# liuzuxin/OSRL

Hardware: AMD Instinct MI355X
Metric: grad-steps/sec (higher is better)
Workload: dtype f32

## Files before the change

### osrl_amd/csrc/mlp.hip

```cpp
#include "dwt.h"
#include "adam.h"
#include "gather.h"
#include "step.h"
#include "trace.h"

namespace {


template <int RW, int CNT, int STAGES, int RD>
__device__ __forceinline__ void mm_prefetch(f32x4 (&b)[RD][RW], int nk, const float* __restrict__ P, int Np, int col0,
                                            int kc0 = 0) {
  static_assert(CNT <= RW && STAGES <= RD, "ring too small");
  const int lane = threadIdx.x & 63;
  const unsigned lane_off = (unsigned)(((lane >> 4) * Np + col0 + (lane & 15)) * 16);
  const int rot = k_rot(nk);
#pragma unroll
  for (int s = 0; s < STAGES - 1; ++s) {
    const int kc = k_at(s < nk ? s : nk - 1, rot, nk, kc0);
    const float* __restrict__ Pk = P + (size_t)kc * 16 * Np;
#pragma unroll
    for (int c = 0; c < CNT; ++c) b[s][c] = load_bp_s(Pk, lane_off + c * 256);
  }
}

// ... 137 lines not shown
__device__ __forceinline__ NarrowPart narrow_part(int nk, int col_off, int nblk, int wave) {
  const int parts = NW / nblk;
  const int blk = wave / parts, part = wave - blk * parts;
  const int k_lo = (nk * part) / parts, k_hi = (nk * (part + 1)) / parts;
  return NarrowPart{col_off + blk * 16, k_lo, k_hi - k_lo};
}
template <int NCB, int NW = 4, int RD = kRing>
__device__ __forceinline__ void narrow_prefetch(f32x4 (&ring)[RD][NCB], int nk, const float* __restrict__ P, int Np,
                                                int col_off, int nblk, int wave) {
  const NarrowPart np = narrow_part<NW>(nk, col_off, nblk, wave);
  if (np.k_n > 0) mm_prefetch<NCB, 1, 3>(ring, np.k_n, P, Np, np.col, np.k_lo);
}
template <int NRB, int NCB, int NW = 4, int RD = kRing>
__device__ __forceinline__ void narrow_layer_splitk(float* lds, int lda, int nk, const float* __restrict__ P, int Np,
                                                    int col_off, int nblk, int wave, f32x4 (&ring)[RD][NCB]) {
  const int lane = threadIdx.x & 63;
  const int parts = NW / nblk;
  const NarrowPart np = narrow_part<NW>(nk, col_off, nblk, wave);
  f32x4 t[NRB][1];
#pragma unroll
  for (int rb = 0; rb < NRB; ++rb) t[rb][0] = f32x4{0.f, 0.f, 0.f, 0.f};
  if (np.k_n > 0) mm_run<NRB, 1, NCB, 1, 3>(lds, lda, np.k_n, P, Np, np.col, t, ring, np.k_lo);
  __syncthreads();
  {
    const int ln = fresh_v<NW == 8>(lane), ld = fresh_s<NW == 8>(lda);
#pragma unroll
    for (int rb = 0; rb < NRB; ++rb)
#pragma unroll
      for (int r = 0; r < 4; ++r) lds[(rb * 16 + (ln >> 4) * 4 + r) * ld + wave * 16 + (ln & 15)] = t[rb][0][r];
  }
  __syncthreads();
  constexpr int BM = 16 * NRB;
  const int ncol = nblk * 16;
  float v[(BM * 32 + 64 * NW - 1) / (64 * NW)];
#pragma unroll
  for (int j = 0; j < (BM * 32 + 64 * NW - 1) / (64 * NW); ++j) {
    const int e = j * 64 * NW + (int)threadIdx.x;
    float sacc = 0.f;
    if (e < BM * ncol) {
      const int r = e / ncol, c = e - r * ncol;
      const int b = c >> 4, cc = c & 15;
      for (int q = 0; q < parts; ++q) sacc += lds[r * lda + (b * parts + q) * 16 + cc];
    }
    v[j] = sacc;
  }
  __syncthreads();
#pragma unroll
  for (int j = 0; j < (BM * 32 + 64 * NW - 1) / (64 * NW); ++j) {
    const int e = j * 64 * NW + (int)threadIdx.x;
    if (e < BM * ncol) {
      const int r = e / ncol, c = e - r * ncol;
      lds[r * lda + c] = v[j];
    }
  }
  __syncthreads();
}


template <int NT = 0>
__device__ __forceinline__ void tile_to_global(const float* lds, int lda, int BM, int N, float* __restrict__ dst,
                                               int row0, int rows) {
  const int tid = threadIdx.x;
  if ((N & 3) == 0 && ((reinterpret_cast<uintptr_t>(dst) & 15) == 0)) {
    const int n4 = N >> 2;
    for (int idx = tid; idx < BM * n4; idx += (NT ? NT : (int)blockDim.x)) {
      const int r = idx / n4, c4 = idx - r * n4;
      if (row0 + r < rows)
        *reinterpret_cast<f32x4*>(dst + (size_t)(row0 + r) * N + 4 * c4) =
            *reinterpret_cast<const f32x4*>(lds + r * lda + 4 * c4);
    }
  } else {
    for (int idx = tid; idx < BM * N; idx += (NT ? NT : (int)blockDim.x)) {
      const int r = idx / N, c = idx - r * N;
      if (row0 + r < rows) dst[(size_t)(row0 + r) * N + c] = lds[r * lda + c];
    }
  }
}

template <int NRB, int NCB, int ACT, bool SCALE, bool RAGGED>
__device__ __forceinline__ void fwd_epilogue_core(float* lds, int lda, const f32x4 (&acc)[NRB][NCB], int cb0, int cnt,
                                                  int N, float oscale, int lane) {
#pragma unroll
  for (int c = 0; c < NCB; ++c) {
    if (c < cnt) {
      const int col = (cb0 + c) * 16 + (lane & 15);
      const bool live = col < N;
      float* dst = lds + ((lane >> 4) * 4) * lda + col;
#pragma unroll
      for (int rb = 0; rb < NRB; ++rb) {
#pragma unroll
        for (int r = 0; r < 4; ++r) {
          float v = act_fwd(ACT, acc[rb][c][r]);
          if (SCALE) v *= oscale;
          if (RAGGED) v = live ? v : 0.f;
          dst[(rb * 16 + r) * lda] = v;
        }
      }
    }
  }
}
template <int NRB, int NCB, int ACT>
__device__ __forceinline__ void fwd_epilogue(float* lds, int lda, const f32x4 (&acc)[NRB][NCB], int cb0, int cnt, int N,
                                             float oscale, int lane) {
  if (oscale == 1.0f && (N & 15) == 0)
    fwd_epilogue_core<NRB, NCB, ACT, false, false>(lds, lda, acc, cb0, cnt, N, oscale, lane);
  else
// ... 41 lines not shown
constexpr float kTailLogStdMin = -20.0f, kTailLogStdMax = 2.0f;
template <class TR, int NT = 0>
__device__ __forceinline__ void tail_gauss(const float* lds, int lda, int BM, int row0, int rows, TR t) {
  const int ad = t.L;
  const float max_a = t.max_action;
  const float* __restrict__ e1 = t.eps;
  const float* __restrict__ e2 = t.eps2;
  float* __restrict__ a1 = t.out;
  float* __restrict__ a2 = t.out2;
  float* __restrict__ th2 = t.tanh2;
  for (int idx = threadIdx.x; idx < BM * ad; idx += (NT ? NT : (int)blockDim.x)) {
    const int r = idx / ad, j = idx - r * ad;
    const int gr = row0 + r;
    if (gr < rows) {
      const float mu = lds[r * lda + j];
      const float ls = fminf(fmaxf(lds[r * lda + ad + j], kTailLogStdMin), kTailLogStdMax);
      const float sd = expf(ls);
      const size_t i = (size_t)gr * ad + j;
      if (e1) {
        const float u = mu + sd * e1[i];
        a1[i] = max_a * tanhf(u);
      }
      if (e2) {
        const float u = mu + sd * e2[i];
        const float th = tanhf(u);
        a2[i] = max_a * th;
        if (th2) th2[i] = th;
      }
    }
  }
  const float* __restrict__ eo = t.eps_ood;
  if (eo) {
    float* __restrict__ so = t.out_ood;
    const int ns = t.n_samples;
    for (int idx = threadIdx.x; idx < ns * BM * ad; idx += (NT ? NT : (int)blockDim.x)) {
      const int jr = idx / ad, k = idx - jr * ad;
      const int smp = jr / BM, r = jr - smp * BM;
      const int gr = row0 + r;
      if (gr < rows) {
        const float mu = lds[r * lda + k];
        const float ls = fminf(fmaxf(lds[r * lda + ad + k], kTailLogStdMin), kTailLogStdMax);
        const size_t i = ((size_t)smp * rows + gr) * ad + k;
        so[i] = mu + expf(ls) * eo[i];
      }
    }
  }
}

struct FwdArgs {
  osrl_mlp_t net;
  osrl_rows_t in;
  osrl_mlp_acts_t out;
  int32_t lda;
  osrl_mlp_tail_t tail;
};

#ifndef OSRL_WPS_8
#define OSRL_WPS_8 3
#endif
constexpr int waves_per_simd(int nrb, int ncb) {
  return nrb * ncb >= 14 ? 2 : nrb * ncb == 8 ? OSRL_WPS_8 : nrb * ncb >= 4 ? 3 : 4;
}
#ifndef OSRL_CHAIN_WPS
#define OSRL_CHAIN_WPS 6
#endif
constexpr int chain_wps(int ncb) { return ncb <= 2 ? OSRL_CHAIN_WPS : 2; }
constexpr int waves_per_simd_bwd(int nrb, int ncb) { return nrb * ncb >= 7 ? 2 : 3; }

template <int NRB, int NCB, int NW, class AR>
__device__ __forceinline__ void mlp_fwd_body(AR a, const int e, const int tile) {
  extern __shared__ __attribute__((aligned(16))) float lds[];
  constexpr int BM = 16 * NRB;
  const int tid = threadIdx.x, lane = tid & 63;
  const int wave = __builtin_amdgcn_readfirstlane(tid >> 6);
  const int row0 = tile * BM;
  const int rows = a.in.rows, lda = a.lda;
  const int L = a.net.n_layers;
#if OSRL_CHAIN_PRIO > 0
  if (rows <= OSRL_CHAIN_PRIO) __builtin_amdgcn_s_setprio(3);
#endif

  WG_LOG(0);
  PHASE_STAMP(0);
  f32x4 ring[ring_depth<NW>()][NCB];
  auto begin_layer = [&](int l) {
    const int K = a.net.dims[l], N = a.net.dims[l + 1];
    const int nblk = (N + 15) >> 4, nk = round16(K) >> 4;
    if (nblk <= 2 && nk >= 4 && lda >= 16 * NW) {
      narrow_prefetch<NCB, NW>(ring, nk, a.net.Wf[e][l], round16(N), 0, nblk, wave);
    } else {
      int cb0, cnt;
      wave_blocks<NW>(nblk, wave, &cb0, &cnt);
      layer_prefetch<NRB, NCB>(ring, nk, a.net.Wf[e][l], round16(N), cb0 * 16, cnt);
    }
  };
  begin_layer(0);
  {
    const int K0 = a.net.dims[0], K0p = round16(K0);
    const int d0 = a.in.d0, d1 = a.in.d1;
    const int cl = tid & 15, rl = tid >> 4;
    const float* __restrict__ s0 = a.in.src0;
    const float* __restrict__ s1 = a.in.src1 ? a.in.src1 : a.in.src0;
#pragma unroll 1
    for (int r = rl; r < BM; r += 4 * NW) {
      const int gr = row0 + r;
      const bool rok = gr < rows;
      const int grc = rok ? gr : rows - 1;
      const float* p0 = s0 + (size_t)map_row(grc, a.in.map0, a.in.div0) * d0;
      const float* p1 = s1 + (size_t)map_row(grc, a.in.map1, a.in.div1) * d1 - d0;
      for (int cbase = 0; cbase < K0p; cbase += 16 * 8) {
        float v[8];
#pragma unroll
        for (int j = 0; j < 8; ++j) {
          const int c = cbase + j * 16 + cl;
          const bool in0 = c < d0, ok = rok && c < d0 + d1;
          const float* p = in0 ? p0 + c : p1 + c;
          v[j] = *(ok ? p : s0);
          v[j] = ok ? v[j] : 0.f;
        }
#pragma unroll
        for (int j = 0; j < 8; ++j) {
          const int c = cbase + j * 16 + cl;
          if (c < K0p) lds[r * lda + c] = v[j];
        }
      }
    }
    __syncthreads();
    if (e == 0 && a.out.x) tile_to_global<64 * NW>(lds, lda, BM, K0, a.out.x, row0, rows);
  }
  PHASE_STAMP(1);
  constexpr bool kWarm = OSRL_L2_WARM && NW == 8;
  float warm[OSRL_MAX_LAYERS - 1][kWarmLines];
  if (kWarm) {
    for (int l = 1; l < L; ++l)
      l2_warm<64 * NW>(a.net.Wf[e][l], round16(a.net.dims[l]) * round16(a.net.dims[l + 1]), warm[l - 1]);
  }

  for (int l = 0; l < L; ++l) {
    const int K = a.net.dims[l], N = a.net.dims[l + 1];
    const int nblk = (N + 15) >> 4;
    const float* __restrict__ bias = a.net.b[e][l];
    const int act = a.net.acts[l];
    const float oscale = (l == L - 1) ? a.net.out_scale : 1.0f;
    const int nk = round16(K) >> 4;
    if (nblk <= 2 && nk >= 4 && lda >= 16 * NW) {
      narrow_layer_splitk<NRB, NCB, NW>(lds, lda, nk, a.net.Wf[e][l], round16(N), 0, nblk, wave, ring);
      if (l + 1 < L) begin_layer(l + 1);
      PHASE_STAMP(2 + 4 * l);
      PHASE_STAMP(3 + 4 * l);
      const int ncol = nblk * 16;
      for (int idx = tid; idx < BM * ncol; idx += 64 * NW) {
        const int r = idx / ncol, c = idx - r * ncol;
        const float v = c < N ? act_fwd(act, lds[r * lda + c] + bias[c]) * oscale : 0.f;
        lds[r * lda + c] = v;
      }
    } else {
      int cb0, cnt;
      wave_blocks<NW>(nblk, wave, &cb0, &cnt);
      float bv[NCB];
#pragma unroll
      for (int c = 0; c < NCB; ++c) {
        const int col = (cb0 + c) * 16 + (lane & 15);
        const bool ok = c < cnt && col < N;
        bv[c] = bias[ok ? col : 0];
        bv[c] = ok ? bv[c] : 0.f;
      }
      f32x4 acc[NRB][NCB];
#pragma unroll
      for (int rb = 0; rb < NRB; ++rb)
#pragma unroll
        for (int c = 0; c < NCB; ++c) acc[rb][c] = f32x4{bv[c], bv[c], bv[c], bv[c]};
      if (cnt > 0) layer_run<NRB, NCB>(lds, lda, nk, a.net.Wf[e][l], round16(N), cb0 * 16, cnt, acc, ring);
      if (l + 1 < L) begin_layer(l + 1);
      PHASE_STAMP(2 + 4 * l);
      __syncthreads();
      PHASE_STAMP(3 + 4 * l);
      const int lane_e = fresh_v<NW == 8>(lane), lda_e = fresh_s<NW == 8>(lda);
      if (act == OSRL_ACT_RELU)
        fwd_epilogue<NRB, NCB, OSRL_ACT_RELU>(lds, lda_e, acc, cb0, cnt, N, oscale, lane_e);
      else if (act == OSRL_ACT_TANH)
        fwd_epilogue<NRB, NCB, OSRL_ACT_TANH>(lds, lda_e, acc, cb0, cnt, N, oscale, lane_e);
      else
        fwd_epilogue<NRB, NCB, OSRL_ACT_ID>(lds, lda_e, acc, cb0, cnt, N, oscale, lane_e);
    }
    PHASE_STAMP(4 + 4 * l);
    __syncthreads();
    float* save = a.out.h[e][l];
    if (save) tile_to_global<64 * NW>(lds, lda, BM, N, save, row0, rows);
    PHASE_STAMP(5 + 4 * l);
    if (kWarm && l == 0) {
      for (int w = 1; w < L; ++w) l2_warm_done(warm[w - 1]);
    }
  }
  if (a.tail.kind == OSRL_TAIL_VAE_LATENT && e == 0) tail_vae_latent<decltype((a.tail)), 64 * NW>(lds, lda, BM, row0, rows, a.tail);
  if (a.tail.kind == OSRL_TAIL_GAUSS && e == 0) tail_gauss<decltype((a.tail)), 64 * NW>(lds, lda, BM, row0, rows, a.tail);
  WG_LOG(1);
}

template <int NRB, int NCB, int NW = 4>
__global__ __launch_bounds__(64 * NW, (NW == 8 ? chain_wps(NCB) : waves_per_simd(NRB, NCB))) void mlp_fwd_kernel(const FwdArgs a) {
  mlp_fwd_body<NRB, NCB, NW, const FwdArgs&>(a, blockIdx.y, blockIdx.x);
}
template <int NRB, int NCB, int NW = 4>
__global__ __launch_bounds__(64 * NW, (NW == 8 ? chain_wps(NCB) : waves_per_simd(NRB, NCB))) void mlp_fwd_kernel_p(const void* p) {
  OSRL_TRACE_BEGIN(5, p);
  mlp_fwd_body<NRB, NCB, NW, const OSRL_CAS FwdArgs&>(*(const OSRL_CAS FwdArgs*)p, blockIdx.y, blockIdx.x);
}

template <int NRB, int NCB>
__global__ __launch_bounds__(256, waves_per_simd(NRB, NCB)) void mlp_fwd_loop_kernel(const FwdArgs a) {
  const int n_tiles = (a.in.rows + 16 * NRB - 1) / (16 * NRB);
  for (int tile = blockIdx.x; tile < n_tiles; tile += gridDim.x) {
    mlp_fwd_body<NRB, NCB, 4, const FwdArgs&>(a, blockIdx.y, tile);
    __syncthreads();
  }
}

struct Fwd2Args {
  FwdArgs a0, a1;
  int32_t nets0, tiles0, tiles1, pad_;
};
template <int NRB, int NCB, int NW = 4>
__global__ __launch_bounds__(64 * NW, (NW == 8 ? chain_wps(NCB) : waves_per_simd(NRB, NCB))) void mlp_fwd2_kernel(
    const Fwd2Args f) {
  if ((int)blockIdx.y < f.nets0) {
    if ((int)blockIdx.x >= f.tiles0) return;
    mlp_fwd_body<NRB, NCB, NW, const FwdArgs&>(f.a0, blockIdx.y, blockIdx.x);
  } else {
    if ((int)blockIdx.x >= f.tiles1) return;
    mlp_fwd_body<NRB, NCB, NW, const FwdArgs&>(f.a1, blockIdx.y - f.nets0, blockIdx.x);
  }
}
template <int NRB, int NCB, int NW = 4>
__global__ __launch_bounds__(64 * NW, (NW == 8 ? chain_wps(NCB) : waves_per_simd(NRB, NCB))) void mlp_fwd2_kernel_p(
    const void* p) {
  OSRL_TRACE_BEGIN(6, p);
  const OSRL_CAS Fwd2Args& f = *(const OSRL_CAS Fwd2Args*)p;
  if ((int)blockIdx.y < f.nets0) {
    if ((int)blockIdx.x >= f.tiles0) return;
    mlp_fwd_body<NRB, NCB, NW, const OSRL_CAS FwdArgs&>(f.a0, blockIdx.y, blockIdx.x);
  } else {
    if ((int)blockIdx.x >= f.tiles1) return;
    mlp_fwd_body<NRB, NCB, NW, const OSRL_CAS FwdArgs&>(f.a1, blockIdx.y - f.nets0, blockIdx.x);
  }
// ... 877 lines not shown
    if (RES) rbase = a.resid + (size_t)urow0 * a.ldr + ucol0;
#pragma unroll
    for (int c = 0; c < CB; ++c) pbias[c] = a.bias ? a.bias[ucol0 + c * 16 + (lane & 15)] : 0.f;
#pragma unroll
    for (int r = 0; r < RB; ++r)
#pragma unroll
      for (int c = 0; c < CB; ++c) {
        prev[r][c] = acc[r][c];
        acc[r][c] = f32x4{0.f, 0.f, 0.f, 0.f};
      }
    tile_ptrs(t + 2 < t1 ? t + 2 : t1 - 1, Agn, Bgn);
  }
#pragma unroll
  for (int e = 0; e < 4 * NACC; ++e) {
    float* yp = ybase + el_off(e, (int)a.ldy);
    const int ai = e >> 2, r = ai % RB, c = ai / RB;
    float v = prev[r][c][e & 3] + pbias[c];
    if (RES) v += (rbase + el_off(e, (int)a.ldr))[loff_r];
    yp[loff_y] = v;
  }
  asm volatile("s_waitcnt vmcnt(0)" ::: "memory");
}


__global__ __launch_bounds__(256) void pack_kernel(const float* __restrict__ src_flat, float* __restrict__ pf,
                                                    float* __restrict__ pb, const osrl_pack_entry_t* __restrict__ ents) {
  const osrl_pack_entry_t E = ents[blockIdx.y];
  const float* __restrict__ W = src_flat + E.src_off;
  const int N = E.out, K = E.in;
  const int Np = round16(N), Kp = round16(K);
  if (pf && E.f_off >= 0) {
    float* __restrict__ d = pf + E.f_off;
    const int total = Kp * Np;
    for (int j = blockIdx.x * 256 + threadIdx.x; j < total; j += gridDim.x * 256) {
      const int t = j & 3, n = (j >> 2) % Np, q = (j >> 2) / Np;
      const int k = q * 4 + t;
      d[j] = (n < N && k < K) ? W[(size_t)n * K + k] : 0.f;
    }
  }
  if (pb && E.b_off >= 0) {
    float* __restrict__ d = pb + E.b_off;
    const int Kb = Kp + 16;
    const int total = Np * Kb;
    for (int j = blockIdx.x * 256 + threadIdx.x; j < total; j += gridDim.x * 256) {
      const int t = j & 3, i = (j >> 2) % Kb, q = (j >> 2) / Kb;
      const int o = q * 4 + t;
      d[j] = (o < N && i < K) ? W[(size_t)o * K + i] : 0.f;
    }
  }
}

inline int round16h(int x) { return (x + 15) & ~15; }

struct TileChoice {
  int nrb, ncb, lda, nw;
};

inline TileChoice choose_tile(const osrl_mlp_t* net, int rows, int extra_width) {
  int maxw = extra_width;
  for (int l = 0; l <= net->n_layers; ++l) maxw = net->dims[l] > maxw ? net->dims[l] : maxw;
  const int nblk = (maxw + 15) / 16;
  const int cpw = (nblk + 3) / 4;
  TileChoice t;
  t.ncb = cpw <= 1 ? 1 : cpw <= 2 ? 2 : cpw <= 4 ? 4 : 7;
  t.lda = round16h(maxw) + 8;
  const long wg32 = (long)((rows + 31) / 32) * net->n_nets;
  t.nrb = (t.ncb != 7 && wg32 >= 1024) ? 2 : 1;
  t.nw = 4;
  if (net->tile_rows == 16 || net->tile_rows == 32 || (net->tile_rows == 64 && t.ncb != 7)) {
    t.nrb = net->tile_rows / 16;
    return t;
  }
  const long wg16 = (long)((rows + 15) / 16) * net->n_nets;
  if (t.nrb == 1 && cpw > 2 && wg16 <= 2 * 256 && t.lda >= 128) {
    t.nw = 8;
    t.ncb = (nblk + 7) / 8 <= 2 ? 2 : 4;
  }
  return t;
}

template <typename Args, typename K>
int launch_tiles(K kernel, void (*kernel_p)(const void*), const Args& args, int rows, int nets, int nrb, int lda,
                 hipStream_t stream, int threads = 256, int wg_cap = 0) {
  const int BM = 16 * nrb;
  const size_t lds_bytes = (size_t)BM * lda * sizeof(float);
  int tiles = (rows + BM - 1) / BM;
  if (wg_cap > 0 && tiles * nets > wg_cap) tiles = (wg_cap + nets - 1) / nets;
  return osrl_argmem::launch(kernel, kernel_p, dim3(tiles, nets, 1), dim3(threads), lds_bytes, stream, args);
}
template <typename Args, typename K>
int launch_tiles(K kernel, const Args& args, int rows, int nets, int nrb, int lda, hipStream_t stream,
                 int threads = 256, int wg_cap = 0) {
  return launch_tiles(kernel, (void (*)(const void*))nullptr, args, rows, nets, nrb, lda, stream, threads, wg_cap);
}

#define OSRL_DISPATCH_TILE(KERNEL, ARGS, ROWS, NETS, T, STREAM, CAP)                        \
  do {                                                                                  \
    if (T.nw == 8) {                                                                    \
      if (T.ncb == 2) return launch_tiles(KERNEL<1, 2, 8>, KERNEL##_p<1, 2, 8>, ARGS, ROWS, NETS, 1, T.lda, STREAM, 512, CAP); \
      return launch_tiles(KERNEL<1, 4, 8>, KERNEL##_p<1, 4, 8>, ARGS, ROWS, NETS, 1, T.lda, STREAM, 512, CAP);     \
    }                                                                                   \
    if (T.ncb == 1) {                                                                   \
      if (T.nrb == 4) return launch_tiles(KERNEL<4, 1>, KERNEL##_p<4, 1>, ARGS, ROWS, NETS, 4, T.lda, STREAM, 256, CAP); \
      if (T.nrb == 2) return launch_tiles(KERNEL<2, 1>, KERNEL##_p<2, 1>, ARGS, ROWS, NETS, 2, T.lda, STREAM, 256, CAP); \
      return launch_tiles(KERNEL<1, 1>, KERNEL##_p<1, 1>, ARGS, ROWS, NETS, 1, T.lda, STREAM, 256, CAP);             \
    }                                                                                   \
    if (T.ncb == 2) {                                                                   \
      if (T.nrb == 4) return launch_tiles(KERNEL<4, 2>, KERNEL##_p<4, 2>, ARGS, ROWS, NETS, 4, T.lda, STREAM, 256, CAP); \
      if (T.nrb == 2) return launch_tiles(KERNEL<2, 2>, KERNEL##_p<2, 2>, ARGS, ROWS, NETS, 2, T.lda, STREAM, 256, CAP); \
      return launch_tiles(KERNEL<1, 2>, KERNEL##_p<1, 2>, ARGS, ROWS, NETS, 1, T.lda, STREAM, 256, CAP);             \
    }                                                                                   \
    if (T.ncb == 4) {                                                                   \
      if (T.nrb == 4) return launch_tiles(KERNEL<4, 4>, KERNEL##_p<4, 4>, ARGS, ROWS, NETS, 4, T.lda, STREAM, 256, CAP); \
      if (T.nrb == 2) return launch_tiles(KERNEL<2, 4>, KERNEL##_p<2, 4>, ARGS, ROWS, NETS, 2, T.lda, STREAM, 256, CAP); \
      return launch_tiles(KERNEL<1, 4>, KERNEL##_p<1, 4>, ARGS, ROWS, NETS, 1, T.lda, STREAM, 256, CAP);             \
    }                                                                                   \
    if (T.nrb == 2) return launch_tiles(KERNEL<2, 7>, KERNEL##_p<2, 7>, ARGS, ROWS, NETS, 2, T.lda, STREAM, 256, CAP); \
    return launch_tiles(KERNEL<1, 7>, KERNEL##_p<1, 7>, ARGS, ROWS, NETS, 1, T.lda, STREAM, 256, CAP);               \
  } while (0)

bool valid_net(const osrl_mlp_t* n) {
  if (!n || n->n_layers < 1 || n->n_layers > OSRL_MAX_LAYERS || n->n_nets < 1 || n->n_nets > OSRL_MAX_NETS)
    return false;
  for (int l = 0; l <= n->n_layers; ++l)
    if (n->dims[l] < 1 || n->dims[l] > OSRL_MAX_WIDTH) return false;
  return true;
}

constexpr int kTileMaxWidth = 448;
bool wide_net(const osrl_mlp_t* n) {
  for (int l = 0; l <= n->n_layers; ++l)
    if (n->dims[l] > kTileMaxWidth) return true;
  return false;
}
enum { WIDE_FWD = 0, WIDE_BWD = 1, WIDE_PLAIN = 2 };
struct WideArgs {
  const float* A[OSRL_MAX_NETS];
  const float* P[OSRL_MAX_NETS];
  const float* bias[OSRL_MAX_NETS];
  const float* h[OSRL_MAX_NETS];
  float* Y[OSRL_MAX_NETS];
  osrl_rows_t in;
  float* x;
  int32_t M, K, N, Np, col0, lda, act, mode;
  float oscale;
};
constexpr int kWideMaxK = OSRL_MAX_WIDTH;
static_assert(sizeof(float) * 16 * (kWideMaxK + 8) <= kLdsMax && sizeof(float) * 32 * (512 + 8) <= kLdsMax,
              "wide_layer_kernel: LDS per workgroup");

template <int NRB, int NCB>
__global__ __launch_bounds__(256) void wide_layer_kernel(const WideArgs a) {
  extern __shared__ __attribute__((aligned(16))) float lds[];
  constexpr int BM = 16 * NRB;
  const int e = blockIdx.z;
  float* __restrict__ Y = a.Y[e];
  if (!Y) return;
  const float* __restrict__ P = a.P[e];
  const int tid = threadIdx.x, lane = tid & 63;
  const int wave = __builtin_amdgcn_readfirstlane(tid >> 6);
  const int row0 = blockIdx.x * BM, M = a.M, K = a.K, N = a.N, lda = a.lda;
  const int Kp = round16(K);
  const int nk = Kp >> 4;
  const int nblk_tot = (N + 15) >> 4;
  constexpr int GB = 4 * NCB;
  const int gb0 = blockIdx.y * GB;
  int nblk = nblk_tot - gb0;
  nblk = nblk > GB ? GB : nblk;
  const bool narrow = nblk_tot <= 2 && nk >= 4 && lda >= 64;
  int cb0 = 0, cnt = 0;
  f32x4 ring[kRing][NCB];
  if (narrow) {
    narrow_prefetch<NCB>(ring, nk, P, a.Np, a.col0, nblk_tot, wave);
  } else {
    wave_blocks(nblk, wave, &cb0, &cnt);
    layer_prefetch<NRB, NCB>(ring, nk, P, a.Np, a.col0 + (gb0 + cb0) * 16, cnt);
  }
  {
    const int cl = tid & 15, rl = tid >> 4;
    const float* __restrict__ A = a.A[e];
    float* __restrict__ x = (a.x && blockIdx.y == 0 && e == 0) ? a.x : nullptr;
    const bool vec = A && (K & 3) == 0 && (reinterpret_cast<uintptr_t>(A) & 15) == 0;
// ... 102 lines not shown
#define STEP_STAMP(i) \
  if (threadIdx.x == 0) g_step_stamp[blockIdx.x][i] = wall_clock64();
#else
#define STEP_STAMP(i)
#endif
constexpr int kStepSpinMax = 1 << 22;
struct StepArgs {
  FwdArgs fwd;
  BwdArgs bwd;
  osrl_gather::GatherArgs gather;
  osrl_step_state_t* st;
  const float* stats_cur;
  float* ring;
  const float* target;
  float* du;
  float* stat;
  const osrl_dw_entry_t* entries;
  const int32_t* work;
  float *p, *m, *v;
  const int32_t *map_f, *map_b;
  float *pf, *pb;
  float* ws;
  float beta1, beta2, lr, eps, inv_n;
  int32_t warmup, n_stats, ring_len, n_tiles, n_work, n_wg, rows, tile_blocks;
};

template <int NCB, class AR>
__device__ __forceinline__ void mlp_step_body(AR a) {
  extern __shared__ __attribute__((aligned(16))) float lds[];
  __shared__ int64_t s_t;
  __shared__ int s_flag;
  __shared__ float s_red[kStepThreads / 64];
  __shared__ float s_part[OSRL_STEP_MAX_WG];
  __shared__ float s_tick[3];
  const int tid = threadIdx.x, lane = tid & 63;
  const int wave = __builtin_amdgcn_readfirstlane(tid >> 6);
  const int wg = blockIdx.x;
  unsigned* __restrict__ ctr = reinterpret_cast<unsigned*>(a.ws + OSRL_STEP_MAX_WG);
  STEP_STAMP(0);
  if (tid == 0) s_t = __atomic_load_n(&a.st->step, __ATOMIC_RELAXED);
  __syncthreads();
  STEP_STAMP(1);
  const int64_t t_old = s_t;
  const uint32_t step = (uint32_t)(t_old + 1);
  if (wg == 0) osrl_step::commit_stats<kStepThreads>(t_old, a.stats_cur, a.ring, a.n_stats, a.ring_len);

  if (wg < a.n_tiles) {
    const int rows = a.rows, row0 = wg * 16;
    if (a.gather.n_fields > 0) {
      osrl_gather::gather_tile16<decltype((a.gather))>(a.gather, step, wg);
      __syncthreads();
    }
    STEP_STAMP(2);
    mlp_fwd_body<1, NCB, 8, decltype((a.fwd))>(a.fwd, 0, wg);
    __syncthreads();
    STEP_STAMP(3);
    {
      const int L = a.fwd.net.n_layers, ad = a.fwd.net.dims[L];
      const float* __restrict__ u = a.fwd.out.h[0][L - 1];
      const float* __restrict__ tg = a.target;
      float* __restrict__ du = a.du;
      const float inv_n = a.inv_n;
      float loss = 0.f;
      int n_here = (rows - row0) * ad;
      n_here = n_here > 16 * ad ? 16 * ad : n_here;
      for (int idx = tid; idx < n_here; idx += kStepThreads) {
        const size_t i = (size_t)row0 * ad + idx;
        const float d = u[i] - tg[i];
        loss += d * d;
        du[i] = 2.0f * d * inv_n;
      }
#pragma unroll
      for (int o = 32; o >= 1; o >>= 1) loss += __shfl_xor(loss, o);
      if (lane == 0) s_red[wave] = loss;
      __syncthreads();
      if (tid == 0)
        a.ws[wg] = (((s_red[0] + s_red[1]) + (s_red[2] + s_red[3])) + ((s_red[4] + s_red[5]) + (s_red[6] + s_red[7])));
    }
    STEP_STAMP(4);
    mlp_bwd_dz_body<1, NCB, 8, decltype((a.bwd))>(a.bwd, 0, wg);
    STEP_STAMP(5);
#if OSRL_STEP_FENCE_ALL
    __threadfence();
    __syncthreads();
    if (tid == 0) {
#else
    asm volatile("s_waitcnt vmcnt(0)" ::: "memory");
    __syncthreads();
    if (tid == 0) {
      __threadfence();
#endif
      const unsigned seen = atomicAdd(ctr, 1u);
      s_flag = seen == (unsigned)a.n_tiles - 1;
      if (s_flag) __threadfence();
    }
    __syncthreads();
    STEP_STAMP(6);
    if (s_flag) {
      if (tid < OSRL_STEP_MAX_WG) s_part[tid] = tid < a.n_tiles ? reinterpret_cast<const volatile float*>(a.ws)[tid] : 0.f;
      __syncthreads();
      if (tid == 0 && a.stat) {
        float t = 0.f;
        for (int g = 0; g < a.n_tiles; ++g) t += s_part[g];
        a.stat[0] = t * a.inv_n;
      }
    }
  }
// ... 204 lines not shown
      a.Y[e] = out->h[e][l];
    }
    if (l == 0) {
      a.in = *in;
      a.x = out->x;
    }
    a.M = in->rows;
    a.K = net->dims[l];
    a.N = net->dims[l + 1];
    a.Np = round16h(a.N);
    a.act = net->acts[l];
    a.mode = WIDE_FWD;
    a.oscale = l == L - 1 ? net->out_scale : 1.0f;
    const int rc = launch_wide_layer(a, E, (hipStream_t)stream);
    if (rc != 0) return rc;
  }
  if (tail && tail->kind != OSRL_TAIL_NONE) return fwd_tail_as_launches(tail, out->h[0][L - 1], in->rows, stream);
  return 0;
}

static int mlp_forward_impl(const osrl_mlp_t* net, const osrl_rows_t* in, const osrl_mlp_acts_t* out,
                            const osrl_mlp_tail_t* tail, void* stream) {
  if (!valid_net(net) || net->out_scale == 0.f || !in || !out || in->rows < 1 || in->d0 + in->d1 != net->dims[0]) return -1;
  for (int e = 0; e < net->n_nets; ++e) {
    if (!out->h[e][net->n_layers - 1]) return -1;
    for (int l = 0; l < net->n_layers; ++l)
      if (!net->Wf[e][l] || !net->b[e][l]) return -1;
  }
  const bool want_tail = tail && tail->kind != OSRL_TAIL_NONE;
  if (want_tail && !fwd_tail_ok(tail, net)) return -1;
  if (wide_net(net)) return mlp_forward_wide(net, in, out, tail, stream);
  {
    const bool kl_tail = want_tail && tail->kind == OSRL_TAIL_VAE_KL;
    const int rc = osrl_launch_fwd_nb(net, in, out, (hipStream_t)stream, kl_tail ? tail->out : nullptr, kl_tail ? tail->L : 0);
    if (rc != kNbNotTaken) {
      if (rc != 0 || !want_tail || kl_tail) return rc;
      if (in->row_list) return -3;
      return fwd_tail_as_launches(tail, out->h[0][net->n_layers - 1], in->rows, stream);
    }
  }
  if (in->row_list || in->n_rows_dev) return -3;
  if (want_tail && tail->kind == OSRL_TAIL_VAE_KL) {
    const int rc = mlp_forward_impl(net, in, out, nullptr, stream);
    return rc != 0 ? rc : fwd_tail_as_launches(tail, out->h[0][net->n_layers - 1], in->rows, stream);
  }
  FwdArgs a{};
  a.net = *net;
  a.in = *in;
  a.out = *out;
  a.tail = osrl_mlp_tail_t{};
  if (want_tail) a.tail = *tail;
  const TileChoice t = choose_tile(net, in->rows, 0);
  a.lda = t.lda;
  if (net->wg_cap > 0 && t.nw == 4 && (t.ncb == 4 || t.ncb == 7) && t.nrb <= 2 &&
      (long)((in->rows + 16 * t.nrb - 1) / (16 * t.nrb)) * net->n_nets > net->wg_cap) {
    hipStream_t st = (hipStream_t)stream;
    const int cap = net->wg_cap, R = in->rows, E = net->n_nets;
    if (t.ncb == 4) {
      if (t.nrb == 2) return launch_tiles(mlp_fwd_loop_kernel<2, 4>, a, R, E, 2, t.lda, st, 256, cap);
      return launch_tiles(mlp_fwd_loop_kernel<1, 4>, a, R, E, 1, t.lda, st, 256, cap);
    }
    if (t.nrb == 2) return launch_tiles(mlp_fwd_loop_kernel<2, 7>, a, R, E, 2, t.lda, st, 256, cap);
    return launch_tiles(mlp_fwd_loop_kernel<1, 7>, a, R, E, 1, t.lda, st, 256, cap);
  }
  OSRL_DISPATCH_TILE(mlp_fwd_kernel, a, in->rows, net->n_nets, t, (hipStream_t)stream, 0);
}

extern "C" int osrl_mlp_forward(const osrl_mlp_t* net, const osrl_rows_t* in, const osrl_mlp_acts_t* out,
                                void* stream) {
  return mlp_forward_impl(net, in, out, nullptr, stream);
}

extern "C" int osrl_mlp_forward_tail(const osrl_mlp_t* net, const osrl_rows_t* in, const osrl_mlp_acts_t* out,
                                     const osrl_mlp_tail_t* tail, void* stream) {
  return mlp_forward_impl(net, in, out, tail, stream);
}

template <int NRB, int NCB, int NW>
static int launch_fwd2(const FwdArgs& a0, const FwdArgs& a1, int nets0, int nets1, int rows0, int rows1, int lda,
                       hipStream_t stream) {
  const int BM = 16 * NRB;
  const int t0 = (rows0 + BM - 1) / BM, t1 = (rows1 + BM - 1) / BM;
  const size_t lds_bytes = (size_t)BM * lda * sizeof(float);
  Fwd2Args f{};
  f.a0 = a0;
  f.a1 = a1;
  f.nets0 = nets0;
  f.tiles0 = t0;
  f.tiles1 = t1;
  return osrl_argmem::launch(mlp_fwd2_kernel<NRB, NCB, NW>, mlp_fwd2_kernel_p<NRB, NCB, NW>,
                             dim3(t0 > t1 ? t0 : t1, nets0 + nets1, 1), dim3(64 * NW), lds_bytes, stream, f);
}

static int mlp_forward2_impl(const osrl_mlp_t* net0, const osrl_rows_t* in0, const osrl_mlp_acts_t* out0,
                             const osrl_mlp_tail_t* tail0, const osrl_mlp_t* net1, const osrl_rows_t* in1,
                             const osrl_mlp_acts_t* out1, const osrl_mlp_tail_t* tail1, void* stream) {
  if (!valid_net(net0) || !valid_net(net1) || !in0 || !in1 || !out0 || !out1) return -1;
  if (in0->row_list || in0->n_rows_dev || in1->row_list || in1->n_rows_dev) return -3;
  if (!fwd_tail_ok(tail0, net0) || !fwd_tail_ok(tail1, net1)) return -1;
  if (wide_net(net0) || wide_net(net1)) {
    const int rc = mlp_forward_impl(net0, in0, out0, tail0, stream);
    return rc != 0 ? rc : mlp_forward_impl(net1, in1, out1, tail1, stream);
  }
  TileChoice t0 = choose_tile(net0, in0->rows, 0), t1 = choose_tile(net1, in1->rows, 0);
  const bool kl_tail = (tail0 && tail0->kind == OSRL_TAIL_VAE_KL) || (tail1 && tail1->kind == OSRL_TAIL_VAE_KL);
  const bool pair = !kl_tail && t0.nrb == 1 && t1.nrb == 1 && t0.ncb == t1.ncb && t0.nw == t1.nw &&
                    ((t0.nw == 8 && (t0.ncb == 2 || t0.ncb == 4)) || (t0.nw == 4 && (t0.ncb == 4 || t0.ncb == 7)));
  if (!pair) {
    const int rc = mlp_forward_impl(net0, in0, out0, tail0, stream);
    return rc != 0 ? rc : mlp_forward_impl(net1, in1, out1, tail1, stream);
  }
  for (int p = 0; p < 2; ++p) {
    const osrl_mlp_t* net = p ? net1 : net0;
    const osrl_rows_t* in = p ? in1 : in0;
    const osrl_mlp_acts_t* out = p ? out1 : out0;
    if (net->out_scale == 0.f || in->rows < 1 || in->d0 + in->d1 != net->dims[0]) return -1;
    for (int e = 0; e < net->n_nets; ++e) {
      if (!out->h[e][net->n_layers - 1]) return -1;
      for (int l = 0; l < net->n_layers; ++l)
        if (!net->Wf[e][l] || !net->b[e][l]) return -1;
    }
  }
  FwdArgs a0{}, a1{};
  a0.net = *net0; a0.in = *in0; a0.out = *out0;
  a1.net = *net1; a1.in = *in1; a1.out = *out1;
  a0.tail = a1.tail = osrl_mlp_tail_t{};
  if (tail0) a0.tail = *tail0;
  if (tail1) a1.tail = *tail1;
  const int lda = t0.lda > t1.lda ? t0.lda : t1.lda;
  a0.lda = a1.lda = lda;
  const int n0 = net0->n_nets, n1 = net1->n_nets, r0 = in0->rows, r1 = in1->rows;
  hipStream_t st = (hipStream_t)stream;
  if (t0.nw == 8) {
    if (t0.ncb == 2) return launch_fwd2<1, 2, 8>(a0, a1, n0, n1, r0, r1, lda, st);
    return launch_fwd2<1, 4, 8>(a0, a1, n0, n1, r0, r1, lda, st);
  }
  if (t0.ncb == 4) return launch_fwd2<1, 4, 4>(a0, a1, n0, n1, r0, r1, lda, st);
  return launch_fwd2<1, 7, 4>(a0, a1, n0, n1, r0, r1, lda, st);
}

extern "C" int osrl_mlp_forward2(const osrl_mlp_t* net0, const osrl_rows_t* in0, const osrl_mlp_acts_t* out0,
                                 const osrl_mlp_t* net1, const osrl_rows_t* in1, const osrl_mlp_acts_t* out1,
                                 void* stream) {
  return mlp_forward2_impl(net0, in0, out0, nullptr, net1, in1, out1, nullptr, stream);
}

extern "C" int osrl_mlp_forward2_tail(const osrl_mlp_t* net0, const osrl_rows_t* in0, const osrl_mlp_acts_t* out0,
                                      const osrl_mlp_tail_t* tail0, const osrl_mlp_t* net1, const osrl_rows_t* in1,
                                      const osrl_mlp_acts_t* out1, const osrl_mlp_tail_t* tail1, void* stream) {
  return mlp_forward2_impl(net0, in0, out0, tail0, net1, in1, out1, tail1, stream);
}

static bool seed_ok(const osrl_mlp_seed_t* s, const osrl_mlp_t* net, const osrl_mlp_acts_t* saved) {
  if (!s || s->kind == OSRL_SEED_NONE) return true;
  const int L = net->n_layers, NL = net->dims[L];
  for (int e = 0; e < net->n_nets; ++e)
    if (!saved->h[e][L - 1]) return false;
  if ((s->partials != nullptr) != (s->counter != nullptr)) return false;
  switch (s->kind) {
    case OSRL_SEED_MSE: return s->x0 && (!s->kl_head || s->kl_L >= 1);
    case OSRL_SEED_CPQ_CRITIC:
      return NL == 1 && s->a && s->b && s->x0 && s->x1 && s->n_a >= 1 && s->n_a <= kSeedEns && s->n_b >= 1 && s->n_b <= kSeedEns;
    case OSRL_SEED_CPQ_COST: return NL == 1 && s->a && s->x0 && s->n_a >= 1 && s->n_a <= kSeedEns;
    case OSRL_SEED_CPQ_ACTOR:
      return NL == 1 && s->a && s->b && s->n_a >= 1 && s->n_a <= kSeedEns && s->n_b >= 1 && s->n_b <= kSeedEns;
    case OSRL_SEED_BCQ_CRITIC:
      return NL == 1 && s->a && s->x0 && s->n_a >= 1 && s->n_b >= 1 && s->n_samples >= 1;
    case OSRL_SEED_FQE:
      return NL == 1 && s->a && s->b && s->x0 && s->x1 && s->n_a >= 1 && s->n_a <= kSeedEns && s->n_b >= 1 && s->n_b <= kSeedEns &&
             s->n_a + s->n_b == net->n_nets && s->kl_head == nullptr;
    case OSRL_SEED_GAUSS_HEAD:
      return (NL & 1) == 0 && net->n_nets == 1 && s->a && s->eps && s->tanh_u && s->n_a >= 1 && s->n_a <= kSeedEns && !s->partials;
    default: return false;
  }
}

static int mlp_backward_dz_impl(const osrl_mlp_t* net, int32_t rows, const osrl_mlp_acts_t* saved,
                                const osrl_mlp_grads_t* g, const osrl_mlp_tail_t* tail, void* stream,
                                const osrl_mlp_seed_t* seed = nullptr);

static int mlp_backward_dz_wide(const osrl_mlp_t* net, int32_t rows, const osrl_mlp_acts_t* saved,
                                const osrl_mlp_grads_t* g, const osrl_mlp_tail_t* tail, void* stream,
                                const osrl_mlp_seed_t* seed) {
// ... 391 lines not shown
```

### osrl_amd/csrc/mlp_common.h

```cpp
#pragma once
#include <hip/hip_runtime.h>
#include <type_traits>
#include <utility>
#include <stdint.h>
#include <stdlib.h>

#include "../../include/osrl_amd.h"
#include "argmem.h"

typedef float f32x4 __attribute__((ext_vector_type(4)));

#if defined(__HIP_DEVICE_COMPILE__) && !defined(__gfx950__)
#error "osrl_amd's in-launch exchanges assume gfx950 memory counters (sc1 stores tracked by vmcnt): build with --offload-arch=gfx950"
#endif

#ifdef OSRL_PHASE_TIMING
__device__ long long g_phase_t[4][64];
__device__ long long g_phase_all[8192][4][16];
#define PHASE_STAMP(i)                                                                                  \
  if ((threadIdx.x & 63) == 0) {                                                                        \
    const long long t_ = __builtin_readcyclecounter();                                                  \
    const int wg_ = blockIdx.x + gridDim.x * blockIdx.y;                                                \
    if (wg_ < 8192 && (i) < 16 && threadIdx.x < 256) g_phase_all[wg_][threadIdx.x >> 6][i] = t_;                             \
    if (blockIdx.x == gridDim.x / 2 && blockIdx.y == 0 && threadIdx.x < 256) g_phase_t[threadIdx.x >> 6][i] = t_;           \
// ... 58 lines not shown
}

__device__ __forceinline__ f32x4 load_bp_s(const float* __restrict__ Pk , unsigned lane_off_bytes) {
#ifdef OSRL_EXP_NO_BLOAD
  const float v = (float)lane_off_bytes * 1e-6f;
  return f32x4{v, v + 1.f, v + 2.f, v + 3.f};
#else
  return *reinterpret_cast<const f32x4*>(reinterpret_cast<const char*>(Pk) + lane_off_bytes);
#endif
}

constexpr int kRing = 3;
#ifndef OSRL_RING_DEEP
#define OSRL_RING_DEEP 3
#endif
constexpr int kRingDeep = OSRL_RING_DEEP;
template <int NW>
constexpr int ring_depth() { return NW == 8 ? kRingDeep : kRing; }
template <class F, int... I>
__device__ __forceinline__ void static_for_impl(F& f, std::integer_sequence<int, I...>) {
  (f(std::integral_constant<int, I>{}), ...);
}
template <int N, class F>
__device__ __forceinline__ void static_for(F&& f) {
  static_for_impl(f, std::make_integer_sequence<int, N>{});
}
constexpr int kWarmLines = 4;
#ifndef OSRL_L2_WARM
#define OSRL_L2_WARM 0
#endif
template <int NT>
__device__ __forceinline__ void l2_warm(const float* __restrict__ P, int n_floats, float (&d)[kWarmLines]) {
  const int n_lines = n_floats >> 5;
#pragma unroll
  for (int j = 0; j < kWarmLines; ++j) {
    int i = (int)threadIdx.x + j * NT;
    i = i < n_lines ? i : n_lines - 1;
    d[j] = P[(size_t)i * 32];
  }
}
__device__ __forceinline__ void l2_warm_done(float (&d)[kWarmLines]) {
#pragma unroll
  for (int j = 0; j < kWarmLines; ++j) asm volatile("" ::"v"(d[j]));
}
#ifndef OSRL_PIN_ROWS
#define OSRL_PIN_ROWS 5
#endif
constexpr int kPinRows = OSRL_PIN_ROWS;

__device__ __forceinline__ int k_rot(int nk) {
  const unsigned w = (unsigned)__builtin_amdgcn_readfirstlane((int)(threadIdx.x >> 6));
  return (int)((blockIdx.x * 5u + blockIdx.y * 3u + w) % (unsigned)nk);
}
__device__ __forceinline__ int k_at(int kc, int rot, int nk, int kc0) {
  const int k = kc + rot;
  return kc0 + (k >= nk ? k - nk : k);
}

#ifdef OSRL_EXP_NO_MFMA
__device__ __forceinline__ f32x4 EXP_MFMA(float a, float b, f32x4 c) {
  c[0] += a * b;
  return c;
}
#else
#define EXP_MFMA(a, b, c) __builtin_amdgcn_mfma_f32_16x16x4f32(a, b, c, 0, 0, 0)
#endif
#ifdef OSRL_EXP_NO_AREAD
#define EXP_AREAD(p) (f32x4{(float)(size_t)(p), 1.f, 2.f, 3.f})
#else
#define EXP_AREAD(p) (*reinterpret_cast<const f32x4*>(p))
#endif

template <int NRB, int NCB>
__device__ __forceinline__ void zero_acc(f32x4 (&acc)[NRB][NCB]) {
#pragma unroll
  for (int rb = 0; rb < NRB; ++rb)
#pragma unroll
    for (int c = 0; c < NCB; ++c) acc[rb][c] = f32x4{0.f, 0.f, 0.f, 0.f};
}

constexpr int kNbNotTaken = -12345;
constexpr size_t kLdsMax = 160 * 1024;
}
__attribute__((visibility("hidden"))) int osrl_launch_fwd_nb(const osrl_mlp_t* net, const osrl_rows_t* in, const osrl_mlp_acts_t* out, hipStream_t stream,
                                                             float* kl = nullptr, int kl_L = 0);
__attribute__((visibility("hidden"))) int osrl_launch_fwd_nb64(const osrl_mlp_t* net, const osrl_rows_t* in, const osrl_mlp_acts_t* out, hipStream_t stream,
                                                             float* kl = nullptr, int kl_L = 0);
```

Baseline: 2506.

## Compute scalar-output head layer with FMA dot products from LDS-parked weights

For 8-wave, single-row-block forward tiles whose last layer has one output, the head weight column is loaded into registers early and parked in extra LDS. The head is then computed as a split-K scalar FMA dot product per row, reduced through padding floats, replacing the MFMA split-K path and its ring prefetch. The aim is less latency on the tiny final layer of critic/value networks. It costs extra LDS per workgroup and adds an env toggle (OSRL_CHAIN_HEAD) that is on by default.

```diff
diff --git a/osrl_amd/csrc/mlp.hip b/osrl_amd/csrc/mlp.hip
--- a/osrl_amd/csrc/mlp.hip
+++ b/osrl_amd/csrc/mlp.hip
@@ -213,6 +213,46 @@
       const int r = e / ncol, c = e - r * ncol;
       lds[r * lda + c] = v[j];
     }
+  }
+  __syncthreads();
+}
+
+constexpr int kChainMaxK = 448;
+template <int NW>
+__device__ __forceinline__ void narrow_layer_chain(float* lds, int lda, int nk, int wave) {
+  static_assert(NW == 8, "one part per wave, one pad float per part");
+  const int tid = fresh_v<true>((int)threadIdx.x), lane = tid & 63;
+  lda = fresh_s<true>(lda);
+  const float* hw = lds + 16 * lda;
+  const int k_lo = (nk * wave) / NW, k_n = (nk * (wave + 1)) / NW - k_lo;
+  float* pad = lds + lda - 8;
+  if (lane < 16) {
+    float acc = 0.f;
+    if (k_n > 0) {
+      const int rot = k_rot_w(k_n, wave);
+      const float* arow = lds + lane * lda;
+      for (int kc = 0; kc < k_n; ++kc) {
+        const int k0 = k_at(kc, rot, k_n, k_lo) * 16;
+        f32x4 av[4], wv[4];
+#pragma unroll
+        for (int kq = 0; kq < 4; ++kq) {
+          av[kq] = *reinterpret_cast<const f32x4*>(arow + k0 + 4 * kq);
+          wv[kq] = *reinterpret_cast<const f32x4*>(hw + k0 + 4 * kq);
+        }
+#pragma unroll
+        for (int t = 0; t < 4; ++t)
+#pragma unroll
+          for (int kq = 0; kq < 4; ++kq) acc = __builtin_fmaf(av[kq][t], wv[kq][t], acc);
+      }
+    }
+    pad[lane * lda + wave] = acc;
+  }
+  __syncthreads();
+  if (tid < 16) {
+    float sacc = 0.f;
+#pragma unroll
+    for (int q = 0; q < NW; ++q) sacc = sacc + pad[tid * lda + q];
+    lds[tid * lda] = sacc;
   }
   __syncthreads();
 }
@@ -360,6 +400,7 @@
   osrl_rows_t in;
   osrl_mlp_acts_t out;
   int32_t lda;
+  int32_t chain_head;
   osrl_mlp_tail_t tail;
 };
 
@@ -375,7 +416,7 @@
 constexpr int chain_wps(int ncb) { return ncb <= 2 ? OSRL_CHAIN_WPS : 2; }
 constexpr int waves_per_simd_bwd(int nrb, int ncb) { return nrb * ncb >= 7 ? 2 : 3; }
 
-template <int NRB, int NCB, int NW, class AR>
+template <int NRB, int NCB, int NW, class AR, bool CH = (NW == 8 && NRB == 1 && NCB <= 2)>
 __device__ __forceinline__ void mlp_fwd_body(AR a, const int e, const int tile) {
   extern __shared__ __attribute__((aligned(16))) float lds[];
   constexpr int BM = 16 * NRB;
@@ -384,6 +425,20 @@
   const int row0 = tile * BM;
   const int rows = a.in.rows, lda = a.lda;
   const int L = a.net.n_layers;
+  bool chain = false;
+  if constexpr (CH) {
+    const int nkh = round16(a.net.dims[L - 1]) >> 4;
+    chain = a.chain_head != 0 && a.net.dims[L] == 1 && nkh >= 4 && 16 * nkh <= kChainMaxK && lda >= 16 * NW;
+  }
+  float hwv = 0.f;
+  auto head_request = [&]() {
+    const int t = fresh_v<CH>(tid);
+    if (CH && chain && t < round16(a.net.dims[L - 1])) hwv = a.net.Wf[e][L - 1][(t >> 2) * 64 + (t & 3)];
+  };
+  auto head_park = [&]() {
+    const int t = fresh_v<CH>(tid);
+    if (CH && chain && t < round16(a.net.dims[L - 1])) lds[BM * fresh_s<CH>(lda) + t] = hwv;
+  };
 #if OSRL_CHAIN_PRIO > 0
   if (rows <= OSRL_CHAIN_PRIO) __builtin_amdgcn_s_setprio(3);
 #endif
@@ -394,6 +449,10 @@
   auto begin_layer = [&](int l) {
     const int K = a.net.dims[l], N = a.net.dims[l + 1];
     const int nblk = (N + 15) >> 4, nk = round16(K) >> 4;
+    if (CH && chain && l == L - 1) {
+      head_request();
+      return;
+    }
     if (nblk <= 2 && nk >= 4 && lda >= 16 * NW) {
       narrow_prefetch<NCB, NW>(ring, nk, a.net.Wf[e][l], round16(N), 0, nblk, wave);
     } else {
@@ -433,6 +492,7 @@
         }
       }
     }
+    if (L == 1) head_park();
     __syncthreads();
     if (e == 0 && a.out.x) tile_to_global<64 * NW>(lds, lda, BM, K0, a.out.x, row0, rows);
   }
@@ -440,7 +500,7 @@
   constexpr bool kWarm = OSRL_L2_WARM && NW == 8;
   float warm[OSRL_MAX_LAYERS - 1][kWarmLines];
   if (kWarm) {
-    for (int l = 1; l < L; ++l)
+    for (int l = 1; l < (CH && chain ? L - 1 : L); ++l)
       l2_warm<64 * NW>(a.net.Wf[e][l], round16(a.net.dims[l]) * round16(a.net.dims[l + 1]), warm[l - 1]);
   }
 
@@ -452,7 +512,14 @@
     const float oscale = (l == L - 1) ? a.net.out_scale : 1.0f;
     const int nk = round16(K) >> 4;
     if (nblk <= 2 && nk >= 4 && lda >= 16 * NW) {
-      narrow_layer_splitk<NRB, NCB, NW>(lds, lda, nk, a.net.Wf[e][l], round16(N), 0, nblk, wave, ring);
+      if constexpr (CH) {
+        if (chain && l == L - 1)
+          narrow_layer_chain<NW>(lds, lda, nk, wave);
+        else
+          narrow_layer_splitk<NRB, NCB, NW>(lds, lda, nk, a.net.Wf[e][l], round16(N), 0, nblk, wave, ring);
+      } else {
+        narrow_layer_splitk<NRB, NCB, NW>(lds, lda, nk, a.net.Wf[e][l], round16(N), 0, nblk, wave, ring);
+      }
       if (l + 1 < L) begin_layer(l + 1);
       PHASE_STAMP(2 + 4 * l);
       PHASE_STAMP(3 + 4 * l);
@@ -492,12 +559,13 @@
         fwd_epilogue<NRB, NCB, OSRL_ACT_ID>(lds, lda_e, acc, cb0, cnt, N, oscale, lane_e);
     }
     PHASE_STAMP(4 + 4 * l);
+    if (l == L - 2) head_park();
     __syncthreads();
     float* save = a.out.h[e][l];
     if (save) tile_to_global<64 * NW>(lds, lda, BM, N, save, row0, rows);
     PHASE_STAMP(5 + 4 * l);
     if (kWarm && l == 0) {
-      for (int w = 1; w < L; ++w) l2_warm_done(warm[w - 1]);
+      for (int w = 1; w < (CH && chain ? L - 1 : L); ++w) l2_warm_done(warm[w - 1]);
     }
   }
   if (a.tail.kind == OSRL_TAIL_VAE_LATENT && e == 0) tail_vae_latent<decltype((a.tail)), 64 * NW>(lds, lda, BM, row0, rows, a.tail);
@@ -1481,6 +1549,11 @@
 
 inline int round16h(int x) { return (x + 15) & ~15; }
 
+inline int chain_head_env() {
+  const char* v = getenv("OSRL_CHAIN_HEAD");
+  return (v && v[0] == '0') ? 0 : 1;
+}
+
 struct TileChoice {
   int nrb, ncb, lda, nw;
 };
@@ -1512,7 +1585,7 @@
 int launch_tiles(K kernel, void (*kernel_p)(const void*), const Args& args, int rows, int nets, int nrb, int lda,
                  hipStream_t stream, int threads = 256, int wg_cap = 0) {
   const int BM = 16 * nrb;
-  const size_t lds_bytes = (size_t)BM * lda * sizeof(float);
+  const size_t lds_bytes = (size_t)BM * lda * sizeof(float) + (threads == 512 ? kChainMaxK * sizeof(float) : 0);
   int tiles = (rows + BM - 1) / BM;
   if (wg_cap > 0 && tiles * nets > wg_cap) tiles = (wg_cap + nets - 1) / nets;
   return osrl_argmem::launch(kernel, kernel_p, dim3(tiles, nets, 1), dim3(threads), lds_bytes, stream, args);
@@ -1557,6 +1630,7 @@
 }
 
 constexpr int kTileMaxWidth = 448;
+static_assert(kTileMaxWidth <= kChainMaxK, "narrow_layer_chain parks the head's weight column in kChainMaxK floats");
 bool wide_net(const osrl_mlp_t* n) {
   for (int l = 0; l <= n->n_layers; ++l)
     if (n->dims[l] > kTileMaxWidth) return true;
@@ -1765,7 +1839,7 @@
       __syncthreads();
     }
     STEP_STAMP(2);
-    mlp_fwd_body<1, NCB, 8, decltype((a.fwd))>(a.fwd, 0, wg);
+    mlp_fwd_body<1, NCB, 8, decltype((a.fwd)), false>(a.fwd, 0, wg);
     __syncthreads();
     STEP_STAMP(3);
     {
@@ -2076,6 +2150,7 @@
   if (want_tail) a.tail = *tail;
   const TileChoice t = choose_tile(net, in->rows, 0);
   a.lda = t.lda;
+  a.chain_head = chain_head_env();
   if (net->wg_cap > 0 && t.nw == 4 && (t.ncb == 4 || t.ncb == 7) && t.nrb <= 2 &&
       (long)((in->rows + 16 * t.nrb - 1) / (16 * t.nrb)) * net->n_nets > net->wg_cap) {
     hipStream_t st = (hipStream_t)stream;
@@ -2105,7 +2180,7 @@
                        hipStream_t stream) {
   const int BM = 16 * NRB;
   const int t0 = (rows0 + BM - 1) / BM, t1 = (rows1 + BM - 1) / BM;
-  const size_t lds_bytes = (size_t)BM * lda * sizeof(float);
+  const size_t lds_bytes = (size_t)BM * lda * sizeof(float) + (NW == 8 ? kChainMaxK * sizeof(float) : 0);
   Fwd2Args f{};
   f.a0 = a0;
   f.a1 = a1;
@@ -2153,6 +2228,7 @@
   if (tail1) a1.tail = *tail1;
   const int lda = t0.lda > t1.lda ? t0.lda : t1.lda;
   a0.lda = a1.lda = lda;
+  a0.chain_head = a1.chain_head = chain_head_env();
   const int n0 = net0->n_nets, n1 = net1->n_nets, r0 = in0->rows, r1 = in1->rows;
   hipStream_t st = (hipStream_t)stream;
   if (t0.nw == 8) {
diff --git a/osrl_amd/csrc/mlp_common.h b/osrl_amd/csrc/mlp_common.h
--- a/osrl_amd/csrc/mlp_common.h
+++ b/osrl_amd/csrc/mlp_common.h
@@ -134,6 +134,9 @@
   const unsigned w = (unsigned)__builtin_amdgcn_readfirstlane((int)(threadIdx.x >> 6));
   return (int)((blockIdx.x * 5u + blockIdx.y * 3u + w) % (unsigned)nk);
 }
+__device__ __forceinline__ int k_rot_w(int nk, int w) {
+  return (int)((blockIdx.x * 5u + blockIdx.y * 3u + (unsigned)w) % (unsigned)nk);
+}
 __device__ __forceinline__ int k_at(int kc, int rot, int nk, int kc0) {
   const int k = kc + rot;
   return kc0 + (k >= nk ? k - nk : k);
```

Measured after the change: 2536, median of 6. 1.01x the previous value.
